# hello-robot/stretch_mujoco

Measured on AMD Instinct MI355X. Metric: env-steps/sec (whole node), 4096 parallel Stretch envs in total, higher is better.
Workload: dtype f32

## Files before the change

stretch_mujoco_amd/csrc/smj_builds.h:

```cpp
#pragma once
#define SMJ_BUILDS_INCLUDED 1

#define SMJ_BUILDS(X) \
  X(step) X(pgs) X(prof) X(tall) X(mid) X(midp) X(big38) X(big38p) X(big50) X(big50p) X(big) X(sat) X(sat1) X(sat2) X(satp) X(sat32) X(sat32n)
#define SMJ_CARRIES_NEWTON 1
#define SMJ_CARRIES_PGS 2
#define SMJ_CARRIES_BOTH 3
#define SMJ_FAM_STD 0
#define SMJ_FAM_TALL 1
#define SMJ_FAM_MID 2
#define SMJ_FAM_BIG38 3
#define SMJ_FAM_BIG50 4
#define SMJ_FAM_BIG 5
#define SMJ_FAM_SAT16 6
#define SMJ_FAM_SAT32 7
#define SMJ_ROW_step    SMJ_FAM_STD,   SMJ_CARRIES_NEWTON, SMJ_CARRIES_NEWTON, 1, 0, 0
#define SMJ_ROW_pgs     SMJ_FAM_STD,   SMJ_CARRIES_PGS,    SMJ_CARRIES_PGS,    1, 0, 0
#define SMJ_ROW_prof    SMJ_FAM_STD,   SMJ_CARRIES_BOTH,   SMJ_CARRIES_BOTH,   1, 0, 1
#define SMJ_ROW_tall    SMJ_FAM_TALL,  SMJ_CARRIES_BOTH,   SMJ_CARRIES_BOTH,   1, 1, 0
#define SMJ_ROW_mid     SMJ_FAM_MID,   SMJ_CARRIES_NEWTON, SMJ_CARRIES_BOTH,   1, 0, 0
#define SMJ_ROW_midp    SMJ_FAM_MID,   SMJ_CARRIES_PGS,    SMJ_CARRIES_PGS,    1, 0, 0
#define SMJ_ROW_big38   SMJ_FAM_BIG38, SMJ_CARRIES_NEWTON, SMJ_CARRIES_BOTH,   1, 0, 0
#define SMJ_ROW_big38p  SMJ_FAM_BIG38, SMJ_CARRIES_PGS,    SMJ_CARRIES_PGS,    1, 0, 0
#define SMJ_ROW_big50   SMJ_FAM_BIG50, SMJ_CARRIES_NEWTON, SMJ_CARRIES_BOTH,   1, 0, 0
#define SMJ_ROW_big50p  SMJ_FAM_BIG50, SMJ_CARRIES_PGS,    SMJ_CARRIES_PGS,    1, 0, 0
#define SMJ_ROW_big     SMJ_FAM_BIG,   SMJ_CARRIES_BOTH,   SMJ_CARRIES_BOTH,   1, 1, 0
#define SMJ_ROW_sat     SMJ_FAM_SAT16, SMJ_CARRIES_NEWTON, SMJ_CARRIES_NEWTON, 1, 0, 0
#define SMJ_ROW_sat1    SMJ_FAM_SAT16, SMJ_CARRIES_PGS,    SMJ_CARRIES_PGS,    1, 0, 0
#define SMJ_ROW_sat2    SMJ_FAM_SAT16, SMJ_CARRIES_NEWTON, SMJ_CARRIES_NEWTON, 2, 0, 0
#define SMJ_ROW_satp    SMJ_FAM_SAT16, SMJ_CARRIES_PGS,    SMJ_CARRIES_PGS,    2, 0, 0
#define SMJ_ROW_sat32   SMJ_FAM_SAT32, SMJ_CARRIES_BOTH,   SMJ_CARRIES_BOTH,   1, 1, 0
#define SMJ_ROW_sat32n  SMJ_FAM_SAT32, SMJ_CARRIES_NEWTON, SMJ_CARRIES_NEWTON, 2, 1, 0
#define smj_step_kernel_step smj_step_kernel
#define smj_launch_step_step smj_launch_step

#define SMJ_CAT2(a, b) a##b
#define SMJ_CAT(a, b) SMJ_CAT2(a, b)
#define SMJ_STR2(a) #a
#define SMJ_STR(a) SMJ_STR2(a)
#define SMJ_COLUMN(m, ...) m(__VA_ARGS__, ~)
#define SMJ_COL0(a, ...) a
#define SMJ_COL1(a, b, ...) b
#define SMJ_COL2(a, b, c, ...) c
#define SMJ_COL3(a, b, c, d, ...) d
#define SMJ_COL4(a, b, c, d, e, ...) e
#define SMJ_COL5(a, b, c, d, e, f, ...) f
#ifdef SMJ_BUILD_TAG
#define SMJ_BUILD_ROW SMJ_CAT(SMJ_ROW_, SMJ_BUILD_TAG)
#define SMJ_BUILD_FAM SMJ_COLUMN(SMJ_COL0, SMJ_BUILD_ROW)
#define SMJ_BUILD_WAVES SMJ_COLUMN(SMJ_COL3, SMJ_BUILD_ROW)
#define SMJ_STEP_KERNEL SMJ_CAT(smj_step_kernel_, SMJ_BUILD_TAG)
#define SMJ_LAUNCH_STEP SMJ_CAT(smj_launch_step_, SMJ_BUILD_TAG)
#if SMJ_COLUMN(SMJ_COL4, SMJ_BUILD_ROW)
#define SMJ_WORKER_KERNEL SMJ_CAT(SMJ_CAT(smj_step_kernel_, SMJ_BUILD_TAG), _worker)
#define SMJ_BUILD_WORKER_NAME SMJ_STR(SMJ_WORKER_KERNEL)
#else
#define SMJ_BUILD_WORKER_NAME nullptr
#endif
#else
#define SMJ_BUILD_FAM SMJ_FAM_STD
#endif

#if SMJ_BUILD_FAM == SMJ_FAM_STD
#define SMJ_BUILD_FAMILY "std"
#elif SMJ_BUILD_FAM == SMJ_FAM_TALL
#define SMJ_BUILD_FAMILY "tall"
#define SMJ_TALL 1
#elif SMJ_BUILD_FAM == SMJ_FAM_MID
#define SMJ_BUILD_FAMILY "mid"
#define SMJ_TALL 1
#define SMJ_TALL_ROWS 128
#define SMJ_TALL_CONTACTS 44
#elif SMJ_BUILD_FAM == SMJ_FAM_BIG38
// ... 84 lines not shown
```

stretch_mujoco_amd/csrc/smj_model.h:

```cpp
#pragma once
#include <stdint.h>

#include "smj_builds.h"
#if defined(SMJ_SAT)
#define NSAT SMJ_SAT
#define NVP 32
#ifndef SMJ_SAT_ROWS
#define SMJ_SAT_ROWS 320
#define SMJ_SAT_CONTACTS 64
#define SMJ_SAT_DENSE 256
#endif
#define NEFC SMJ_SAT_ROWS
#define NCON SMJ_SAT_CONTACTS
#define NDR SMJ_SAT_DENSE
#ifndef SMJ_SAT_EXT
#define SMJ_SAT_EXT 4
#endif
#ifndef SMJ_SAT_PGS
#define SMJ_SAT_PGS (SMJ_SAT_DENSE < 160 ? SMJ_SAT_DENSE : 160)
#endif
#define NXS SMJ_SAT_EXT
static_assert(NDR % 16 == 0 && NDR <= NEFC, "dense rows: whole 16-row blocks (matT_J, MFMA k-steps)");
#define NENT 5
#elif defined(SMJ_BIG)
// ... 87 lines not shown
  int nsat, nq_all, nv_all, nbody_all, nfric_main, nlimit_main;
  const int* k_satrec;
  int nsgeom, nstatpair, grid_dim[3];
  float grid_org[3], grid_h, grid_margin;
  const int* k_sgrec;
  const int* k_sprec;
  const int* k_spair;
  const int* k_grid_adr;
  const int* k_grid_list;
  const int* k_sg_cell;
  const float* k_sg_bound;
  const float* k_sgw;
#define X(n) const int* n;
  SMJ_MODEL_I32(X)
#undef X
#define X(n) const float* n;
  SMJ_MODEL_F32(X)
#undef X
  const int* k_lanerec;
  const int* k_pprec;
  const int* k_cgrec;
  const int* k_rowrec;
  const int* k_cprec;
};
enum { SMJ_CP_PAIR = 0, SMJ_CP_G1, SMJ_CP_G2, SMJ_CP_S1, SMJ_CP_S2, SMJ_CP_MARGIN, SMJ_CP_MG, SMJ_CP_CONDIM, SMJ_CP_FRIC = 8, SMJ_CP_SOLIMP = 13,
       SMJ_CP_SOLREF = 18, SMJ_CP_RBMIN = 20 ,
       SMJ_CP_B1 = 21, SMJ_CP_B2 = 22 , SMJ_CP_STRIDE = 24 };
enum { SMJ_RR_TYPE = 0, SMJ_RR_ID, SMJ_RR_D1, SMJ_RR_D2, SMJ_RR_Q1, SMJ_RR_Q2, SMJ_RR_V1, SMJ_RR_V2, SMJ_RR_DATA = 8, SMJ_RR_DIAG = 13,
       SMJ_RR_FLOSS = 14, SMJ_RR_SOLREF = 15, SMJ_RR_SOLIMP = 17, SMJ_RR_SAT = 22 , SMJ_RR_SDOF = 23 , SMJ_RR_STRIDE = 24 };
constexpr int smj_lr_act(int nent) { return 76 + ((7 * nent + 3) & ~3); }
constexpr int smj_lr_stride(int nent) { return smj_lr_act(nent) + 28; }
enum { SMJ_LR_KIN = 0, SMJ_LR_BODY = 36, SMJ_LR_DOF = 60, SMJ_LR_ENT = 76, SMJ_LR_ACT = smj_lr_act(NENT), SMJ_LR_STRIDE = smj_lr_stride(NENT) };
enum { SMJ_PP_PAIR = 0, SMJ_PP_G1, SMJ_PP_G2, SMJ_PP_B1, SMJ_PP_B2, SMJ_PP_T2, SMJ_PP_MARGIN, SMJ_PP_RBOUND2, SMJ_PP_BCEN2 = 8,
       SMJ_PP_POS1 = 11, SMJ_PP_MAT1 = 14, SMJ_PP_POS2 = 23, SMJ_PP_MAT2 = 26, SMJ_PP_SIZE2 = 35, SMJ_PP_CONDIM = 38, SMJ_PP_MG = 39,
       SMJ_PP_FRIC = 40, SMJ_PP_SOLIMP = 45, SMJ_PP_SOLREF = 50, SMJ_PP_BOX2 = 52 ,
       SMJ_PP_STRIDE = 60 };
enum { SMJ_CG_GEOM = 0, SMJ_CG_BODY, SMJ_CG_META, SMJ_CG_POS = 3, SMJ_CG_MAT = 6, SMJ_CG_LCEN = 15, SMJ_CG_HALF = 18, SMJ_CG_CCEN = 21,
       SMJ_CG_SIZE = 24, SMJ_CG_RBOUND = 27, SMJ_CG_STRIDE = 28 };

enum { SMJ_SR_BODY = 0, SMJ_SR_JTYPE, SMJ_SR_QADR, SMJ_SR_DADR, SMJ_SR_NDOF, SMJ_SR_JNT, SMJ_SR_F = 8,
       SMJ_SR_POS = SMJ_SR_F + 0, SMJ_SR_QUAT = SMJ_SR_F + 3, SMJ_SR_JPOS = SMJ_SR_F + 7, SMJ_SR_JAXIS = SMJ_SR_F + 10, SMJ_SR_Q0 = SMJ_SR_F + 13,
       SMJ_SR_INL = SMJ_SR_F + 14, SMJ_SR_ARM = SMJ_SR_F + 24, SMJ_SR_DAMP = SMJ_SR_F + 30, SMJ_SR_STIFF = SMJ_SR_F + 36, SMJ_SR_SPRING = SMJ_SR_F + 37,
       SMJ_SR_GCMASS = SMJ_SR_F + 38, SMJ_SR_GCIPOS = SMJ_SR_F + 39, SMJ_SR_STRIDE = 52 };
struct SmjStageLayout {
  int qpos, qvel, warm, ctrl, bctl, nstep, info, actlen, actvel, base, gyro, accel, xpose, stride;
};
constexpr SmjStageLayout smj_stage_layout(int nvp, int nbp, int nsat = 0) {
// ... 99 lines not shown
```

stretch_mujoco_amd/csrc/smj_model_load.h:

```cpp
#pragma once
#include <stdint.h>
#include <stdio.h>
#include <math.h>
#include <string.h>

#include <map>
#include <string>
#include <vector>

#include "../../include/smj.h"
#include "smj_model.h"

#define SMJ_SOLVER_OPTIONS(X)                                                                                                             \
  X("iterations", iterations, int) X("tolerance", tolerance, float) X("warmstart", warmstart, int) X("pgs_fixed_iter", pgs_fixed_iter, int) \
  X("qcqp_exact", qcqp_exact, int) X("grad_noise", grad_noise, float) X("pgs_island_stop", pgs_island_stop, int)                            \
  X("max_contacts_per_pair", max_con_pair, int) X("solver", solver, int) X("convex_pairs", convex_pairs, int) X("multiccd", multiccd, int)  \
  X("sep_cache", sep_cache, int) X("manifold_cache", manifold_cache, int) X("pgs_dual_warmstart", pgs_dual_ws, int)                         \
  X("", ls_iterations, int) X("", multi_serial, int) X("", ls_tolerance, float)
static inline bool smj_set_solver_option(DevModel& m, const char* name, double v) {
#define X(opt, field, type) if ((opt)[0] && !strcmp(name, opt)) { m.field = (type)v; return true; }
  SMJ_SOLVER_OPTIONS(X)
#undef X
  return false;
}
// ... 108 lines not shown
      for (int u = 0; u < nent; u++) {
        const int e = L + 64 * u, ok = e < m.nldl, ex = ok ? e : 0, i = gi("k_ldl_i", ex), j = gi("k_ldl_j", ex);
        k[u] = ok ? i : -1; k[nent + u] = ok ? j : 0; k[2 * nent + u] = fb((ok && i == j) ? gf("dof_armature", i) : 0.f);
        k[3 * nent + u] = ok ? gi("k_ldl_lact", ex) : -1;
        k[4 * nent + u] = fb(ok ? gf("k_ldl_damp", ex) : 0.f); k[5 * nent + u] = fb(ok ? gf("k_ldl_dcoef", ex) : 0.f); k[6 * nent + u] = fb(ok ? gf("k_ldl_lcoef", ex) : 0.f);
      }
    }
    {
      int* k = r + LR_ACT;
      const int a = L < nu ? L : 0;
      for (int u = 0; u < 4; u++) {
        const int dd = gi("k_act_dof", 4 * a + u);
        k[u] = L < nu ? dd : -1; k[4 + u] = dd >= 0 ? gi("k_dof_qposadr", dd) : 0; k[8 + u] = fb(gf("k_act_mom", 4 * a + u));
      }
      k[12] = fb(gf("actuator_gainprm", 3 * a));
      for (int q = 0; q < 3; q++) k[13 + q] = fb(gf("actuator_biasprm", 3 * a + q));
      k[16] = fb(gf("actuator_ctrlrange", 2 * a)); k[17] = fb(gf("actuator_ctrlrange", 2 * a + 1));
      k[18] = fb(gf("actuator_forcerange", 2 * a)); k[19] = fb(gf("actuator_forcerange", 2 * a + 1));
      k[20] = (gi("actuator_ctrllimited", a) ? 1 : 0) | (gi("actuator_forcelimited", a) ? 2 : 0) | (gi("actuator_biastype", a) == 1 ? 4 : 0);
      const int g = L < m.ngc ? gi("k_gc_body", L) : 0;
      k[21] = g; k[22] = gi("k_body_dofmask_lo", g); k[23] = gi("k_body_dofmask_hi", g);
      k[24] = fb(L < m.ngc ? gf("body_gcmass", g) : 0.f);
      for (int q = 0; q < 3; q++) k[25 + q] = fb(gf("body_gcipos", 3 * g + q));
    }
  }
  return rec;
}

static inline std::vector<int> smj_build_pprec(const DevModel& m, std::map<std::string, std::vector<int>>& I,
                                               std::map<std::string, std::vector<float>>& F) {
  std::vector<int> rec((size_t)(m.nplanepair > 0 ? m.nplanepair : 1) * SMJ_PP_STRIDE, 0);
  auto fb = [](float v) { int b; memcpy(&b, &v, 4); return b; };
  auto gi = [&](const char* n, size_t k) { const std::vector<int>& v = I[n]; return k < v.size() ? v[k] : 0; };
  auto gf = [&](const char* n, size_t k) { const std::vector<float>& v = F[n]; return k < v.size() ? v[k] : 0.f; };
  for (int t = 0; t < m.nplanepair; t++) {
    int* k = rec.data() + (size_t)t * SMJ_PP_STRIDE;
    const int p = gi("k_planepair", t), g1 = gi("pair_geom1", p), g2 = gi("pair_geom2", p);
    k[SMJ_PP_PAIR] = p; k[SMJ_PP_G1] = g1; k[SMJ_PP_G2] = g2; k[SMJ_PP_B1] = gi("geom_bodyid", g1); k[SMJ_PP_B2] = gi("geom_bodyid", g2);
    k[SMJ_PP_T2] = gi("geom_type", g2); k[SMJ_PP_MARGIN] = fb(gf("pair_margin", p)); k[SMJ_PP_RBOUND2] = fb(gf("geom_rbound", g2));
    for (int q = 0; q < 3; q++) {
      k[SMJ_PP_BCEN2 + q] = fb(gf("k_geom_bcenter", 3 * g2 + q));
      k[SMJ_PP_POS1 + q] = fb(gf("geom_pos", 3 * g1 + q)); k[SMJ_PP_POS2 + q] = fb(gf("geom_pos", 3 * g2 + q));
      k[SMJ_PP_SIZE2 + q] = fb(gf("geom_size", 3 * g2 + q));
    }
    for (int q = 0; q < 9; q++) { k[SMJ_PP_MAT1 + q] = fb(gf("k_geom_mat", 9 * g1 + q)); k[SMJ_PP_MAT2 + q] = fb(gf("k_geom_mat", 9 * g2 + q)); }
    k[SMJ_PP_CONDIM] = gi("pair_condim", p); k[SMJ_PP_MG] = fb(gf("pair_margin", p) - gf("pair_gap", p));
// ... 266 lines not shown
    const SmjBlobEntry* ei = b.find("k_sat_i");
    const SmjBlobEntry* ef = b.find("k_sat_f");
    if (!ei || !ef || ei->dtype != 1 || ef->dtype != 0 || ei->nbytes < 32u * m.nsat || ef->nbytes < 8u * 44u * m.nsat) { err = "model blob: satellite tables missing"; return -3; }
    std::vector<int> si(8 * (size_t)m.nsat), rec((size_t)m.nsat * SMJ_SR_STRIDE, 0);
    memcpy(si.data(), b.p + ei->offset, 32u * m.nsat);
    hosti["k_sat_i"] = si;
    const double* sf = reinterpret_cast<const double*>(b.p + ef->offset);
    for (int sidx = 0; sidx < m.nsat; sidx++) {
      int* k = rec.data() + (size_t)sidx * SMJ_SR_STRIDE;
      for (int q = 0; q < 8; q++) k[q] = si[8 * sidx + q];
      for (int q = 0; q < 44; q++) { const float v = (float)sf[44 * sidx + q]; memcpy(&k[SMJ_SR_F + q], &v, 4); }
    }
    m.k_satrec = up.i32(rec);
    if (!m.k_satrec) { err = "device allocation failed for k_satrec"; return -2; }
    m.nfric_main = 0;
    for (int f = 0; f < m.nfric; f++) m.nfric_main += hosti["k_fric_dof"][f] < m.nv;
    m.nlimit_main = 0;
    for (int L = 0; L < m.nlimit; L++) m.nlimit_main += hosti["jnt_dofadr"][hosti["k_limit_jnt"][L]] < m.nv;
  }
  {
    std::vector<int> rec = smj_build_lanerec(m, hosti, hostf, nent);
    m.k_lanerec = up.i32(rec);
    if (!m.k_lanerec) { err = "device allocation failed for k_lanerec"; return -2; }
    std::vector<int> pp = smj_build_pprec(m, hosti, hostf), cg = smj_build_cgrec(m, hosti, hostf);
    m.k_pprec = up.i32(pp);
    m.k_cgrec = up.i32(cg);
    if (!m.k_pprec || !m.k_cgrec) { err = "device allocation failed for the collision records"; return -2; }
    std::vector<int> rr = smj_build_rowrec(m, hosti, hostf);
    m.k_rowrec = up.i32(rr);
    if (!m.k_rowrec) { err = "device allocation failed for k_rowrec"; return -2; }
    std::vector<int> cp = smj_build_cprec(m, hosti, hostf);
    m.k_cprec = up.i32(cp);
    if (!m.k_cprec) { err = "device allocation failed for k_cprec"; return -2; }
  }
  return 0;
}
```

stretch_mujoco_amd/csrc/smj_step_impl.h:

```cpp
#pragma once
#ifndef SMJ_PROFILING
#define SMJ_PROFILING 1
#endif
#include <cstddef>
#include "smj_model.h"
#include "smj_wave.h"
#include "smj_sat_mem.h"

#define JS (NVS + 1)
#define MS (NVS + 1)
#define SMJ_MINVAL 1e-15f
#define SMJ_MINIMP 0.0001f
#define SMJ_MAXIMP 0.9999f

enum { JT_FREE = 0, JT_BALL = 1, JT_SLIDE = 2, JT_HINGE = 3 };
enum { GT_PLANE = 0, GT_SPHERE = 2, GT_CAPSULE = 3, GT_ELLIPSOID = 4, GT_CYLINDER = 5, GT_BOX = 6, GT_MESH = 7 };
enum { CT_EQUALITY = 0, CT_FRICTION = 1, CT_LIMIT = 3, CT_CONTACT_FRICTIONLESS = 5, CT_CONTACT_ELLIPTIC = 7, CT_NONE = -1 };

#if NSAT > 0
#define NCGS (NCG + 1)
#define NSURV 128
#else
#define NCGS NCG
#endif
// ... 239 lines not shown
    la = fmaxf(0.f, la + delta);
  }
#pragma unroll
  for (int i = 0; i < N; i++) res[i] *= dd[i];
  la_io = la;
  return la != 0;
}

SMJ_DEV float impedance(const float* solimp, float pos, float margin) {
  float dmin = fminf(SMJ_MAXIMP, fmaxf(SMJ_MINIMP, solimp[0])), dmax = fminf(SMJ_MAXIMP, fmaxf(SMJ_MINIMP, solimp[1]));
  float width = fmaxf(SMJ_MINVAL, solimp[2]), mid = fminf(SMJ_MAXIMP, fmaxf(SMJ_MINIMP, solimp[3])), power = fmaxf(1.0f, solimp[4]);
  if (dmin == dmax) return 0.5f * (dmin + dmax);
  float x = fabsf(pos - margin) / width, y;
  if (x >= 1) return dmax;
  if (x <= 0) return dmin;
  if (power == 1.0f) y = x;
  else if (power == 2.0f) y = (x <= mid) ? x * x / mid : 1 - (1 - x) * (1 - x) / (1 - mid);
  else if (x <= mid) y = powf(x, power) / powf(mid, power - 1);
  else y = 1 - powf(1 - x, power) / powf(1 - mid, power - 1);
  return dmin + y * (dmax - dmin);
}

#ifdef SMJ_EMUL
static long smj_emul_sep_skips = 0;
static long smj_emul_ext_steps = 0;
static long smj_emul_mc_hits = 0;
static long smj_emul_isl_total = 0, smj_emul_isl_swept = 0;
#endif
struct StepKernel {
  const DevModel& M;
  const DevState& S;
  Smem& s;
  int env;

  PL<float[6]> cdof, cdof_dot;
  PL<float> qvel_r, g_r, qacc_r;
  PL<float> f_r[NPS], r_r[NPS], ARinv_r[NPS];
  PL<float> qla_r;
  int nefc, ncon, niter, flags;
  float* ppc = nullptr;
  int step_base = 0;
  int pipe_chunk = 0;
  bool parked = false;
  bool split_on = false, rev = false;
  bool serial_redo = false;

// ... 3121 lines not shown
    LANES { if (lane == 0) s.sat.nch = 0; }
#endif
    SYNC();
    ROWS_BEGIN(rb, ne) LANES {
      float c = 0, f = 0;
      int st = 0;
      const int i = lane + rb, t = nr.type[lane];
      const float jar = nr.jar[lane], D = nr.D[lane], R = nr.R[lane];
      if (i < ne) {
        if (t == CT_EQUALITY) { f = -D * jar; st = 1; c = 0.5f * D * jar * jar; }
        else if (t == CT_FRICTION) {
          const float fl = nr.fl[lane];
          if (jar <= -R * fl) { f = fl; st = 2; c = -fl * (0.5f * R * fl + jar); }
          else if (jar >= R * fl) { f = -fl; st = 3; c = -fl * (0.5f * R * fl - jar); }
          else { f = -D * jar; st = 1; c = 0.5f * D * jar * jar; }
        } else if (t == CT_LIMIT || t == CT_CONTACT_FRICTIONLESS) {
          if (jar < 0) { f = -D * jar; st = 1; c = 0.5f * D * jar * jar; }
        }
      }
      nr.force[lane] = f; nr.state[lane] = st; cost[lane] += c;
      if (i < NEFC) s.ef[i] = f;
    } ROWS_END_RW(rb)
    SYNC();
    ROWS_BEGIN(rb, ne) LANES {
      const int c = nr.c0[lane];
      if (c >= 0) {
        const int i = lane + rb, dim = s.cdim[c];
        const float mu = nr.cq[lane][6];
        float U[6], jr[6], S[6], Rj[6], T = 0;
#pragma unroll
        for (int j = 0; j < 6; j++) {
          const int jj = j < dim ? j : 0;
          jr[j] = s.eb[i + jj];
          Rj[j] = s.eR[i + jj];
          S[j] = j == 0 ? mu : (j < dim ? s.cfric[c][j - 1] : 0.f);
          U[j] = jr[j] * S[j];
          if (j > 0) T += U[j] * U[j];
        }
        const float N = U[0];
        const float Tinv = T > 0 ? fast_rsqrt(T) : 0.f;
        T = T * Tinv;
        int st;
        float cc = 0, ef[6] = {0, 0, 0, 0, 0, 0};
        if (N >= mu * T || (T <= 0 && N >= 0)) { st = 0; }
        else if (mu * N + T <= 0 || (T <= 0 && N < 0)) {
          st = 1;
#pragma unroll
          for (int j = 0; j < 6; j++)
            if (j < dim) { const float Dj = fast_rcp(Rj[j]); ef[j] = -Dj * jr[j]; cc += 0.5f * Dj * jr[j] * jr[j]; }
        } else {
          st = 4;
          const float Dm = nr.cq[lane][5], NT = N - mu * T, Ti = Tinv;
          cc = 0.5f * Dm * NT * NT;
          const float fn = -Dm * NT * mu;
          ef[0] = fn;
#pragma unroll
          for (int j = 1; j < 6; j++) ef[j] = -fn * Ti * U[j] * S[j];
#if NSAT > 0
          const int hslot = want_hess ? lds_atomic_inc(&s.sat.nch) : NCH;
          s.sat.chs[c] = hslot < NCH ? (signed char)hslot : (signed char)-1;
          if (want_hess && hslot < NCH) {
            float* H = s.u.n.cH[hslot];
#else
          if (want_hess) {
            float* H = s.u.n.cH[c];
#endif
            const float a = mu * N * Ti * Ti * Ti, b = mu * NT * Ti;
            H[0] = Dm * S[0] * S[0];
#pragma unroll
            for (int j = 1; j < 6; j++) H[j] = H[6 * j] = -mu * U[j] * Ti * Dm * S[0] * S[j];
#pragma unroll
            for (int j = 1; j < 6; j++)
#pragma unroll
              for (int k = 1; k < 6; k++) H[6 * j + k] = (a * U[j] * U[k] - (j == k ? b : 0.f)) * Dm * S[j] * S[k];
          }
        }
        cost[lane] += cc;
#pragma unroll
        for (int j = 0; j < 6; j++)
          if (j < dim) { s.ef[i + j] = ef[j]; s.estate[i + j] = st; }
      }
    } ROWS_END_RO()
    SYNC();
    ROWS_BEGIN(rb, ne) LANES {
      const int i = lane + rb;
      if (i < NEFC) {
        if (nr.type[lane] == CT_CONTACT_ELLIPTIC && i < ne) { nr.force[lane] = s.ef[i]; nr.state[lane] = s.estate[i]; }
        s.estate[i] = (i < ne) ? nr.state[lane] : 0;
      }
    } ROWS_END_RW(rb)
    return wave_sum(cost);
  }

#ifdef SMJ_EMUL
  struct F2 { float x, y; };
  static inline void pk_fma(F2& acc, float a0, float a1, float b0, float b1) { acc.x += a0 * b0; acc.y += a1 * b1; }
#else
  typedef float F2 __attribute__((ext_vector_type(2)));
  SMJ_DEV static void pk_fma(F2& acc, float a0, float a1, float b0, float b1) {
    const F2 a = {a0, a1}, b = {b0, b1};
    acc = acc + a * b;
  }
#endif
// ... 147 lines not shown
    } else if constexpr (J < N) {
      PL<float> cj;
      LANES { cj[lane] = hrow[lane][J]; }
      const float hkj = wave_read(cj, K);
      LANES { hrow[lane][J] -= mult[lane] * hkj; }
    }
  }
  template <int K, int N>
  SMJ_DEV void gj_cols(PL<float[NVS]>& hrow, PL<float>& x, PL<float>& pinv, const PL<int>& ol) {
    if constexpr (K < N) {
      PL<float> col, mult;
      LANES { col[lane] = hrow[lane][K]; }
      const float rp = fast_rcp(fmaxf(wave_read(col, K), 1e-30f));
      LANES {
        mult[lane] = ol[lane] == K ? 0.f : col[lane] * rp;
        if (ol[lane] == K) pinv[lane] = rp;
      }
      gj_pair<K, K + 1, N>(hrow, mult);
      const float xk = wave_read(x, K);
      LANES { x[lane] -= mult[lane] * xk; }
      gj_cols<K + 1, N>(hrow, x, pinv, ol);
    }
  }
  template <int N>
  SMJ_DEV void gj_solve(PL<float>& x) {
    PL<float[NVS]> hrow;
    PL<float> pinv;
    PL<int> ol;
    LANES { ol[lane] = opaque(lane); }
    LANES {
      const int i = NVS == 32 ? (lane & 31) : (lane < NVS ? lane : NVS - 1);
#pragma unroll
      for (int k = 0; k < N; k++) hrow[lane][k] = s.u.n.H[i][k];
      pinv[lane] = 0.f;
      if (lane >= N) x[lane] = 0.f;
    }
    gj_cols<0, N>(hrow, x, pinv, ol);
    LANES { x[lane] *= pinv[lane]; }
  }
  SMJ_DEV void gj_solve_lds(PL<float>& x) {
    const int n = M.nv;
    LANES { if (lane < NVS) s.u.n.H[lane][NVS] = lane < n ? x[lane] : 0.f; }
    SYNC();
    for (int k = 0; k < n; k++) {
      const float rp = fast_rcp(fmaxf(uni(s.u.n.H[k][k]), 1e-30f));
      LANES {
        if (lane < n && lane != k) {
          float* row = s.u.n.H[lane];
          const float* piv = s.u.n.H[k];
          const float mult = row[k] * rp;
          int j = k + 1;
          for (; j + 8 <= n; j += 8) {
            float a[8], b[8];
#pragma unroll
            for (int u = 0; u < 8; u++) { a[u] = row[j + u]; b[u] = piv[j + u]; }
#pragma unroll
            for (int u = 0; u < 8; u++) row[j + u] = a[u] - mult * b[u];
          }
          for (; j < n; j++) row[j] -= mult * piv[j];
          row[NVS] -= mult * piv[NVS];
        }
      }
      SYNC();
    }
    LANES { x[lane] = lane < n ? s.u.n.H[lane][NVS] * fast_rcp(fmaxf(s.u.n.H[lane][lane], 1e-30f)) : 0.f; }
    SYNC();
  }
  SMJ_DEV void solve_H(PL<float>& x, bool rare = false) {
#if NVP == 32
    if (M.nv <= 26) gj_solve<26>(x);
    else gj_solve<NVP>(x);
#else
    if (rare || M.nv > 50) gj_solve_lds(x);
#if NVS >= 50
    else if (M.nv > 38) gj_solve<50>(x);
#endif
    else gj_solve<38>(x);
#endif
  }

  SMJ_DEV float ls_eval(NRow& nr0, const float* qg, float a, float& d1, float& d2) {
    const int ne = nefc;
    PL<float> p0, p1, p2;
    LANES { p0[lane] = 0.f; p1[lane] = 0.f; p2[lane] = 0.f; }
    ROWS_BEGIN(rb, ne) LANES {
      float c0 = 0, c1 = 0, c2 = 0;
      if (lane + rb < ne) {
        const int t = nr.type[lane];
        const float x = nr.jar[lane] + a * nr.jv[lane];
        if (t == CT_EQUALITY) { c0 = nr.q0[lane]; c1 = nr.q1[lane]; c2 = nr.q2[lane]; }
        else if (t == CT_FRICTION) {
          const float fl = nr.fl[lane], rf = nr.R[lane] * fl;
          if (x <= -rf) { c0 = fl * (-0.5f * rf - nr.jar[lane]); c1 = -fl * nr.jv[lane]; }
          else if (x >= rf) { c0 = fl * (-0.5f * rf + nr.jar[lane]); c1 = fl * nr.jv[lane]; }
          else { c0 = nr.q0[lane]; c1 = nr.q1[lane]; c2 = nr.q2[lane]; }
        } else if (t == CT_LIMIT || t == CT_CONTACT_FRICTIONLESS) {
          if (x < 0) { c0 = nr.q0[lane]; c1 = nr.q1[lane]; c2 = nr.q2[lane]; }
        } else if (nr.c0[lane] >= 0) {
          const float* k = nr.cq[lane];
          const float mu = k[6], Dm = k[5], N = k[0] + a * k[1], Tsq = k[2] + a * (2 * k[3] + a * k[4]);
          if (Tsq <= 0) { if (N < 0) { c0 = nr.q0[lane]; c1 = nr.q1[lane]; c2 = nr.q2[lane]; } }
          else {
            const float Ti = fast_rsqrt(Tsq), T = Tsq * Ti;
            if (N >= mu * T) {}
            else if (mu * N + T <= 0) { c0 = nr.q0[lane]; c1 = nr.q1[lane]; c2 = nr.q2[lane]; }
            else {
              const float w = k[3] + a * k[4], N1 = k[1], T1 = w * Ti, T2 = k[4] * Ti - w * w * Ti * Ti * Ti;
              const float NT = N - mu * T, NT1 = N1 - mu * T1;
              const float v = 0.5f * Dm * NT * NT, g = Dm * NT * NT1, h = Dm * (NT1 * NT1 - NT * mu * T2);
              c2 = 0.5f * h; c1 = g - h * a; c0 = v - a * g + 0.5f * h * a * a;
            }
          }
        }
      }
      p0[lane] += c0; p1[lane] += c1; p2[lane] += c2;
    } ROWS_END_RO()
    const float q0 = qg[0] + wave_sum(p0), q1 = qg[1] + wave_sum(p1), q2 = qg[2] + wave_sum(p2);
    d1 = 2 * a * q2 + q1;
    d2 = 2 * q2;
    return a * a * q2 + a * q1 + q0;
  }
// ... 22 lines not shown
#endif
      }
      niter = 0;
      SYNC();
      return;
    }
    ROWS_BEGIN_(rb, ne, false) LANES {
      const int row = lane + rb;
      float vel = 0;
      const bool on = row < ne;
      if (on) {
        const float* jr = jrow(row);
        for (int k = 0; k < nv; k++) vel += jr[k] * s.qvel[k];
#if NSAT > 0
        vel += sat_jdot(row, SX_V);
#endif
      }
      nr.type[lane] = on ? s.etype[row] : CT_NONE;
      nr.R[lane] = on ? s.eR[row] : 1.f;
      nr.D[lane] = on ? 1.0f / s.eR[row] : 0.f;
      nr.fl[lane] = on ? s.efloss[row] : 0.f;
      nr.aref[lane] = on ? -s.eBv[row] * vel - s.eK[row] * s.eimp[row] * (s.epos[row] - s.emargin[row]) : 0.f;
      int c0 = -1;
      if (on && s.etype[row] == CT_CONTACT_ELLIPTIC && s.cefc[s.eid[row]] == row) c0 = s.eid[row];
      nr.c0[lane] = c0;
      nr.state[lane] = 0; nr.jar[lane] = 0.f; nr.jv[lane] = 0.f; nr.force[lane] = 0.f; nr.q0[lane] = 0.f; nr.q1[lane] = 0.f; nr.q2[lane] = 0.f;
      for (int k = 0; k < 7; k++) nr.cq[lane][k] = 0.f;
      if (c0 >= 0) {
        const float mu = contact_mu(c0);
        nr.cq[lane][6] = mu;
        nr.cq[lane][5] = (1.0f / s.eR[row]) / fmaxf(mu * mu * (1 + mu * mu), SMJ_MINVAL);
      }
      if (dbg && row < NEFC) s.earef[row] = nr.aref[lane];
    } ROWS_END_RW(rb)
#if NSAT > 0
    const int nvt = M.nv_all;
#else
    const int nvt = nv;
#endif
    const float scale = 1.0f / (M.meaninertia * (float)(nvt > 1 ? nvt : 1));
    LANES { qacc[lane] = (lane < nv && M.warmstart) ? s.warm[lane] : 0.f; }
    mat_M(Ma, qacc);
#if NSAT > 0
    if (!M.warmstart) { LANES { if (lane >= 32 && lane - 32 < M.nsat) for (int k = 0; k < 6; k++) s.sat.x[SX_QA][lane - 32][k] = 0.f; } }
    sat_matM(SX_MA, SX_QA);
    SYNC();
#endif
    ROWS_BEGIN(rb, ne) mat_J_exact(nr.jar, qacc, nr.aref, rb); ROWS_END_RW(rb)
    float cost = 0;
    TICK(SMJ_PROF_WARM)
    int iter = 0;
    bool at_update = false;
    for (; iter < M.iterations;) {
      TICK(SMJ_PROF_PGS)
// ... 91 lines not shown
                  for (int t = 0; t < NT; t++) b[t][lane][ks] = s.J[k][16 * t + c];
                }
              }
            }
#pragma unroll
            for (int ks = 0; ks < KB; ks++) {
              if (kb + ks < ksteps && kb + ks < NDR / 4) {
                PL<float> pa[NT], pb[NT];
                LANES {
#pragma unroll
                  for (int t = 0; t < NT; t++) { pb[t][lane] = b[t][lane][ks]; pa[t][lane] = wk[lane][ks] * pb[t][lane]; }
                }
#pragma unroll
                for (int ta = 0; ta < NT; ta++)
#pragma unroll
                  for (int tb = 0; tb <= ta; tb++) mfma16x16x4(acc[ta * (ta + 1) / 2 + tb], pa[ta], pb[tb]);
              }
            }
          }
        }
        long long th = 0;
        if (prof) { th = smj_clock(); pc[SMJ_PROF_H_K] += (float)(th - t0); }
        int nks = 0;
        for (uint64_t cm = conemask; cm;) {
          const int c = ffs64(cm);
          cm &= cm - 1;
          const int r0 = uni(s.cefc[c]), dim = uni(s.cdim[c]);
          if (r0 >= ndense()) continue;
          for (int q0 = 0; q0 < dim; q0 += 4) {
            nks++;
            PL<float> pa[NT], pb[NT];
            LANES {
              const int q = q0 + (lane >> 4), col = lane & 15, qc = q < 6 ? q : 5;
              const float on = q < dim ? 1.f : 0.f;
              float hq[6];
#if NSAT > 0
              const int hc = s.sat.chs[c];
#else
              const int hc = c;
#endif
#pragma unroll
              for (int p = 0; p < 6; p++) hq[p] = on * s.u.n.cH[hc][6 * qc + p];
#pragma unroll
              for (int t = 0; t < NT; t++) {
                float jv[6], av = 0.f;
#pragma unroll
// ... 88 lines not shown
          a1[lane] = lane < nv ? search[lane] * (Ma[lane] - g_r[lane]) : 0.f;
          a2[lane] = lane < nv ? 0.5f * search[lane] * Mv[lane] : 0.f;
#if NSAT > 0
          if (lane >= 32 && lane - 32 < M.nsat) {
            const int si = lane - 32;
            for (int k = 0; k < 6; k++) {
              a1[lane] += s.sat.x[SX_SRCH][si][k] * (s.sat.x[SX_MA][si][k] - s.sat.x[SX_G][si][k]);
              a2[lane] += 0.5f * s.sat.x[SX_SRCH][si][k] * s.sat.x[SX_MV][si][k];
            }
          }
#endif
        }
        qg[0] = gauss; qg[1] = wave_sum(a1); qg[2] = wave_sum(a2);
      }
      ROWS_BEGIN(rb, ne) LANES {
        const int row = lane + rb;
        const float D = nr.D[lane], ja = nr.jar[lane], jv = nr.jv[lane];
        nr.q0[lane] = 0.5f * D * ja * ja; nr.q1[lane] = D * ja * jv; nr.q2[lane] = 0.5f * D * jv * jv;
        if (row < NEFC) { s.eb[row] = ja; s.ef[row] = jv; s.earef[row] = nr.q0[lane]; s.eK[row] = nr.q1[lane]; s.eBv[row] = nr.q2[lane]; }
      } ROWS_END_RW(rb)
      SYNC();
      ROWS_BEGIN(rb, ne) LANES {
        const int c = nr.c0[lane];
        if (c >= 0) {
          const int i = lane + rb, dim = s.cdim[c];
          float a0 = 0, a1 = 0, a2 = 0, uu = 0, uv = 0, vv = 0;
#pragma unroll
          for (int j = 1; j < 6; j++) {
            const int jj = j < dim ? j : 1;
            const float on = j < dim ? 1.f : 0.f;
            a0 += on * s.earef[i + jj]; a1 += on * s.eK[i + jj]; a2 += on * s.eBv[i + jj];
            const float fr = on * s.cfric[c][jj - 1], u = s.eb[i + jj] * fr, v = s.ef[i + jj] * fr;
            uu += u * u; uv += u * v; vv += v * v;
          }
          nr.q0[lane] += a0; nr.q1[lane] += a1; nr.q2[lane] += a2;
          const float mu = nr.cq[lane][6];
          nr.cq[lane][0] = nr.jar[lane] * mu; nr.cq[lane][1] = nr.jv[lane] * mu;
          nr.cq[lane][2] = uu; nr.cq[lane][3] = uv; nr.cq[lane][4] = vv;
        }
      } ROWS_END_RW(rb)
      TICK(SMJ_PROF_N_PREP)
      float alpha = 0, d10 = 0;
      {
        const float gtol = M.tolerance * M.ls_tolerance * snorm * M.meaninertia * (float)(nvt > 1 ? nvt : 1);
        float d1, d2, lo = 0, hi = -1;
        {
          PL<float> gs;
// ... 97 lines not shown
      for (int t = 0; t < NENT; t++) {
        const int i = et.i[lane][t], j = et.j[lane][t];
        if (i < 0) continue;
        float v = (i == j) ? s.Mdiag[i] : s.MM[j][i];
        if (implicit) {
          float d = et.damp[lane][t] - et.dcoef[lane][t];
          const int la = et.lact[lane][t];
          if (la >= 0) d -= et.lcoef[lane][t] * s.act_free[la];
          v += h * d;
        }
        s.u.n.H[i][j] = v;
        s.u.n.H[j][i] = v;
      }
    }
    SYNC();
  }

  SMJ_DEV void integrate() {
    const int nv = M.nv;
    const float h = M.timestep;
#if SMJ_W2_INTEGRATE
    fork2(W2_SAT_INTEGRATE);
#endif
    build_dense(true);
    PL<float> x;
    LANES { x[lane] = lane < nv ? s.tmp[lane] : 0.f; }
    solve_H(x);
    LANES {
      if (lane < nv) s.qvel[lane] += h * x[lane];
    }
    SYNC();
    LANES {
      if (lane < M.njnt) {
        const int j = lane, qa = M.jnt_qposadr[j], da = M.jnt_dofadr[j];
        if (M.jnt_type[j] == JT_FREE) {
          for (int k = 0; k < 3; k++) s.qpos[qa + k] += h * s.qvel[da + k];
          float wv[3] = {s.qvel[da + 3], s.qvel[da + 4], s.qvel[da + 5]};
          const float nrm = sqrtf(dot3(wv, wv)), ang = nrm * h;
          float q[4] = {s.qpos[qa + 3], s.qpos[qa + 4], s.qpos[qa + 5], s.qpos[qa + 6]};
          if (ang > 0) {
            const float sn = sinf(0.5f * ang) / nrm, dq[4] = {cosf(0.5f * ang), wv[0] * sn, wv[1] * sn, wv[2] * sn};
            quat_mul(q, q, dq);
          }
          quat_normalize(q);
          for (int k = 0; k < 4; k++) s.qpos[qa + 3 + k] = q[k];
        } else s.qpos[qa] += h * s.qvel[da];
      }
    }
    SYNC();
    PL<int> bad;
// ... 248 lines not shown
```

Measured before the change: 12.97 million.

## Batch cone Hessian MFMA k-steps across contacts, fill cone Hessian by rows, direct-integrate from MM

Adds a per-build cone-batch column (set to 4 for step, prof and mid). When it is above one, the Newton cone-Hessian accumulation gathers several contacts per group and issues their MFMA k-steps together, instead of looping one contact at a time. The cone Hessian blocks are filled in parallel by friction rows (encoding row index in c0), rather than one lane writing all 36 entries. Integration can skip build_dense by patching only the implicit damping entries of the mass matrix in place, solving from it, and restoring them, driven by a new host-built per-row sparse record. This adds register pressure, more complex encoding, and a new device table.

```diff
diff --git a/stretch_mujoco_amd/csrc/smj_builds.h b/stretch_mujoco_amd/csrc/smj_builds.h
--- a/stretch_mujoco_amd/csrc/smj_builds.h
+++ b/stretch_mujoco_amd/csrc/smj_builds.h
@@ -14,23 +14,23 @@
 #define SMJ_FAM_BIG 5
 #define SMJ_FAM_SAT16 6
 #define SMJ_FAM_SAT32 7
-#define SMJ_ROW_step    SMJ_FAM_STD,   SMJ_CARRIES_NEWTON, SMJ_CARRIES_NEWTON, 1, 0, 0
-#define SMJ_ROW_pgs     SMJ_FAM_STD,   SMJ_CARRIES_PGS,    SMJ_CARRIES_PGS,    1, 0, 0
-#define SMJ_ROW_prof    SMJ_FAM_STD,   SMJ_CARRIES_BOTH,   SMJ_CARRIES_BOTH,   1, 0, 1
-#define SMJ_ROW_tall    SMJ_FAM_TALL,  SMJ_CARRIES_BOTH,   SMJ_CARRIES_BOTH,   1, 1, 0
-#define SMJ_ROW_mid     SMJ_FAM_MID,   SMJ_CARRIES_NEWTON, SMJ_CARRIES_BOTH,   1, 0, 0
-#define SMJ_ROW_midp    SMJ_FAM_MID,   SMJ_CARRIES_PGS,    SMJ_CARRIES_PGS,    1, 0, 0
-#define SMJ_ROW_big38   SMJ_FAM_BIG38, SMJ_CARRIES_NEWTON, SMJ_CARRIES_BOTH,   1, 0, 0
-#define SMJ_ROW_big38p  SMJ_FAM_BIG38, SMJ_CARRIES_PGS,    SMJ_CARRIES_PGS,    1, 0, 0
-#define SMJ_ROW_big50   SMJ_FAM_BIG50, SMJ_CARRIES_NEWTON, SMJ_CARRIES_BOTH,   1, 0, 0
-#define SMJ_ROW_big50p  SMJ_FAM_BIG50, SMJ_CARRIES_PGS,    SMJ_CARRIES_PGS,    1, 0, 0
-#define SMJ_ROW_big     SMJ_FAM_BIG,   SMJ_CARRIES_BOTH,   SMJ_CARRIES_BOTH,   1, 1, 0
-#define SMJ_ROW_sat     SMJ_FAM_SAT16, SMJ_CARRIES_NEWTON, SMJ_CARRIES_NEWTON, 1, 0, 0
-#define SMJ_ROW_sat1    SMJ_FAM_SAT16, SMJ_CARRIES_PGS,    SMJ_CARRIES_PGS,    1, 0, 0
-#define SMJ_ROW_sat2    SMJ_FAM_SAT16, SMJ_CARRIES_NEWTON, SMJ_CARRIES_NEWTON, 2, 0, 0
-#define SMJ_ROW_satp    SMJ_FAM_SAT16, SMJ_CARRIES_PGS,    SMJ_CARRIES_PGS,    2, 0, 0
-#define SMJ_ROW_sat32   SMJ_FAM_SAT32, SMJ_CARRIES_BOTH,   SMJ_CARRIES_BOTH,   1, 1, 0
-#define SMJ_ROW_sat32n  SMJ_FAM_SAT32, SMJ_CARRIES_NEWTON, SMJ_CARRIES_NEWTON, 2, 1, 0
+#define SMJ_ROW_step    SMJ_FAM_STD,   SMJ_CARRIES_NEWTON, SMJ_CARRIES_NEWTON, 1, 0, 0, 4
+#define SMJ_ROW_pgs     SMJ_FAM_STD,   SMJ_CARRIES_PGS,    SMJ_CARRIES_PGS,    1, 0, 0, 1
+#define SMJ_ROW_prof    SMJ_FAM_STD,   SMJ_CARRIES_BOTH,   SMJ_CARRIES_BOTH,   1, 0, 1, 4
+#define SMJ_ROW_tall    SMJ_FAM_TALL,  SMJ_CARRIES_BOTH,   SMJ_CARRIES_BOTH,   1, 1, 0, 1
+#define SMJ_ROW_mid     SMJ_FAM_MID,   SMJ_CARRIES_NEWTON, SMJ_CARRIES_BOTH,   1, 0, 0, 4
+#define SMJ_ROW_midp    SMJ_FAM_MID,   SMJ_CARRIES_PGS,    SMJ_CARRIES_PGS,    1, 0, 0, 1
+#define SMJ_ROW_big38   SMJ_FAM_BIG38, SMJ_CARRIES_NEWTON, SMJ_CARRIES_BOTH,   1, 0, 0, 1
+#define SMJ_ROW_big38p  SMJ_FAM_BIG38, SMJ_CARRIES_PGS,    SMJ_CARRIES_PGS,    1, 0, 0, 1
+#define SMJ_ROW_big50   SMJ_FAM_BIG50, SMJ_CARRIES_NEWTON, SMJ_CARRIES_BOTH,   1, 0, 0, 1
+#define SMJ_ROW_big50p  SMJ_FAM_BIG50, SMJ_CARRIES_PGS,    SMJ_CARRIES_PGS,    1, 0, 0, 1
+#define SMJ_ROW_big     SMJ_FAM_BIG,   SMJ_CARRIES_BOTH,   SMJ_CARRIES_BOTH,   1, 1, 0, 1
+#define SMJ_ROW_sat     SMJ_FAM_SAT16, SMJ_CARRIES_NEWTON, SMJ_CARRIES_NEWTON, 1, 0, 0, 1
+#define SMJ_ROW_sat1    SMJ_FAM_SAT16, SMJ_CARRIES_PGS,    SMJ_CARRIES_PGS,    1, 0, 0, 1
+#define SMJ_ROW_sat2    SMJ_FAM_SAT16, SMJ_CARRIES_NEWTON, SMJ_CARRIES_NEWTON, 2, 0, 0, 1
+#define SMJ_ROW_satp    SMJ_FAM_SAT16, SMJ_CARRIES_PGS,    SMJ_CARRIES_PGS,    2, 0, 0, 1
+#define SMJ_ROW_sat32   SMJ_FAM_SAT32, SMJ_CARRIES_BOTH,   SMJ_CARRIES_BOTH,   1, 1, 0, 1
+#define SMJ_ROW_sat32n  SMJ_FAM_SAT32, SMJ_CARRIES_NEWTON, SMJ_CARRIES_NEWTON, 2, 1, 0, 1
 #define smj_step_kernel_step smj_step_kernel
 #define smj_launch_step_step smj_launch_step
 
@@ -45,10 +45,14 @@
 #define SMJ_COL3(a, b, c, d, ...) d
 #define SMJ_COL4(a, b, c, d, e, ...) e
 #define SMJ_COL5(a, b, c, d, e, f, ...) f
+#define SMJ_COL6(a, b, c, d, e, f, g, ...) g
 #ifdef SMJ_BUILD_TAG
 #define SMJ_BUILD_ROW SMJ_CAT(SMJ_ROW_, SMJ_BUILD_TAG)
 #define SMJ_BUILD_FAM SMJ_COLUMN(SMJ_COL0, SMJ_BUILD_ROW)
 #define SMJ_BUILD_WAVES SMJ_COLUMN(SMJ_COL3, SMJ_BUILD_ROW)
+#ifndef SMJ_CONE_CB
+#define SMJ_CONE_CB SMJ_COLUMN(SMJ_COL6, SMJ_BUILD_ROW)
+#endif
 #define SMJ_STEP_KERNEL SMJ_CAT(smj_step_kernel_, SMJ_BUILD_TAG)
 #define SMJ_LAUNCH_STEP SMJ_CAT(smj_launch_step_, SMJ_BUILD_TAG)
 #if SMJ_COLUMN(SMJ_COL4, SMJ_BUILD_ROW)
diff --git a/stretch_mujoco_amd/csrc/smj_model.h b/stretch_mujoco_amd/csrc/smj_model.h
--- a/stretch_mujoco_amd/csrc/smj_model.h
+++ b/stretch_mujoco_amd/csrc/smj_model.h
@@ -133,7 +133,10 @@
   const int* k_cgrec;
   const int* k_rowrec;
   const int* k_cprec;
-};
+  const int* k_imprec;
+  int imp_nslot;
+};
+enum { SMJ_IR_N = 8, SMJ_IR_STRIDE = 5 * SMJ_IR_N };
 enum { SMJ_CP_PAIR = 0, SMJ_CP_G1, SMJ_CP_G2, SMJ_CP_S1, SMJ_CP_S2, SMJ_CP_MARGIN, SMJ_CP_MG, SMJ_CP_CONDIM, SMJ_CP_FRIC = 8, SMJ_CP_SOLIMP = 13,
        SMJ_CP_SOLREF = 18, SMJ_CP_RBMIN = 20 ,
        SMJ_CP_B1 = 21, SMJ_CP_B2 = 22 , SMJ_CP_STRIDE = 24 };
diff --git a/stretch_mujoco_amd/csrc/smj_model_load.h b/stretch_mujoco_amd/csrc/smj_model_load.h
--- a/stretch_mujoco_amd/csrc/smj_model_load.h
+++ b/stretch_mujoco_amd/csrc/smj_model_load.h
@@ -154,6 +154,31 @@
       k[21] = g; k[22] = gi("k_body_dofmask_lo", g); k[23] = gi("k_body_dofmask_hi", g);
       k[24] = fb(L < m.ngc ? gf("body_gcmass", g) : 0.f);
       for (int q = 0; q < 3; q++) k[25 + q] = fb(gf("body_gcipos", 3 * g + q));
+    }
+  }
+  return rec;
+}
+
+static inline std::vector<int> smj_build_imprec(const DevModel& m, std::map<std::string, std::vector<int>>& I,
+                                                std::map<std::string, std::vector<float>>& F, int& nslot) {
+  std::vector<int> rec(64 * SMJ_IR_STRIDE, 0);
+  auto fb = [](float v) { int b; memcpy(&b, &v, 4); return b; };
+  auto gi = [&](const char* n, size_t k) { const std::vector<int>& v = I[n]; return k < v.size() ? v[k] : 0; };
+  auto gf = [&](const char* n, size_t k) { const std::vector<float>& v = F[n]; return k < v.size() ? v[k] : 0.f; };
+  for (int L = 0; L < 64; L++)
+    for (int u = 0; u < SMJ_IR_N; u++) { rec[L * SMJ_IR_STRIDE + u] = -1; rec[L * SMJ_IR_STRIDE + SMJ_IR_N + u] = -1; }
+  int used[64] = {0};
+  nslot = 0;
+  for (int e = 0; e < m.nldl; e++) {
+    const int i = gi("k_ldl_i", e), j = gi("k_ldl_j", e), la = gi("k_ldl_lact", e);
+    const float damp = gf("k_ldl_damp", e), dcoef = gf("k_ldl_dcoef", e), lcoef = gf("k_ldl_lcoef", e);
+    if (damp == 0.f && dcoef == 0.f && la < 0) continue;
+    for (int side = 0; side < (i == j ? 1 : 2); side++) {
+      const int row = side ? j : i, col = side ? i : j;
+      if (row < 0 || row >= m.nv || row >= 64 || used[row] >= SMJ_IR_N) { nslot = -1; return rec; }
+      int* k = rec.data() + row * SMJ_IR_STRIDE + used[row]++;
+      k[0] = col; k[SMJ_IR_N] = la; k[2 * SMJ_IR_N] = fb(damp); k[3 * SMJ_IR_N] = fb(dcoef); k[4 * SMJ_IR_N] = fb(lcoef);
+      if (used[row] > nslot) nslot = used[row];
     }
   }
   return rec;
@@ -466,6 +491,9 @@
     std::vector<int> rec = smj_build_lanerec(m, hosti, hostf, nent);
     m.k_lanerec = up.i32(rec);
     if (!m.k_lanerec) { err = "device allocation failed for k_lanerec"; return -2; }
+    std::vector<int> ir = smj_build_imprec(m, hosti, hostf, m.imp_nslot);
+    m.k_imprec = up.i32(ir);
+    if (!m.k_imprec) { err = "device allocation failed for k_imprec"; return -2; }
     std::vector<int> pp = smj_build_pprec(m, hosti, hostf), cg = smj_build_cgrec(m, hosti, hostf);
     m.k_pprec = up.i32(pp);
     m.k_cgrec = up.i32(cg);
diff --git a/stretch_mujoco_amd/csrc/smj_step_impl.h b/stretch_mujoco_amd/csrc/smj_step_impl.h
--- a/stretch_mujoco_amd/csrc/smj_step_impl.h
+++ b/stretch_mujoco_amd/csrc/smj_step_impl.h
@@ -285,6 +285,21 @@
 }
 
 #ifdef SMJ_EMUL
+#undef SMJ_CONE_CB
+#define SMJ_CONE_CB (NVP == 32 ? 4 : 2)
+#elif !defined(SMJ_CONE_CB)
+#define SMJ_CONE_CB 1
+#endif
+static_assert(SMJ_CONE_CB == 1 || SMJ_CONE_CB % 2 == 0, "a group is whole contacts: two k-steps each");
+#define SMJ_NEWTON_BATCHED (SMJ_CONE_CB > 1)
+#define SMJ_CH_ROWS (SMJ_NEWTON_BATCHED && NSAT == 0)
+#ifdef SMJ_EMUL
+extern "C" {
+int smj_emul_serial_newton = 0;
+long smj_emul_cone_group_ksteps = 0;
+long smj_emul_ch_row_fills = 0;
+long smj_emul_direct_integrations = 0;
+}
 static long smj_emul_sep_skips = 0;
 static long smj_emul_ext_steps = 0;
 static long smj_emul_mc_hits = 0;
@@ -3452,11 +3467,17 @@
       if (i < NEFC) s.ef[i] = f;
     } ROWS_END_RW(rb)
     SYNC();
+#if SMJ_CH_ROWS && defined(SMJ_EMUL)
+    const bool by_rows = want_hess && !smj_emul_serial_newton;
+#else
+    const bool by_rows = SMJ_CH_ROWS && want_hess;
+#endif
     ROWS_BEGIN(rb, ne) LANES {
-      const int c = nr.c0[lane];
-      if (c >= 0) {
-        const int i = lane + rb, dim = s.cdim[c];
+      const int cj = nr.c0[lane];
+      if (cj >= 0 && (cj < 256 || by_rows)) {
+        const int c = cj & 255, j = cj >> 8, i = lane + rb - j, dim = s.cdim[c];
         const float mu = nr.cq[lane][6];
+        const float So = j == 0 ? mu : s.cfric[c][j > 0 ? j - 1 : 0], Uo = s.eb[lane + rb < NEFC ? lane + rb : 0] * So;
         float U[6], jr[6], S[6], Rj[6], T = 0;
 #pragma unroll
         for (int j = 0; j < 6; j++) {
@@ -3496,6 +3517,21 @@
             float* H = s.u.n.cH[c];
 #endif
             const float a = mu * N * Ti * Ti * Ti, b = mu * NT * Ti;
+#if SMJ_CH_ROWS
+            if (by_rows) {
+#ifdef SMJ_EMUL
+              smj_emul_ch_row_fills++;
+#endif
+              H[6 * j] = j == 0 ? Dm * S[0] * S[0] : -mu * Uo * Ti * Dm * S[0] * So;
+#pragma unroll
+              for (int k = 1; k < 6; k++)
+                H[6 * j + k] = j == 0 ? -mu * U[k] * Ti * Dm * S[0] * S[k] : (a * Uo * U[k] - (j == k ? b : 0.f)) * Dm * So * S[k];
+              if (j + dim < 6)
+#pragma unroll
+                for (int k = 0; k < 6; k++) H[6 * (j + dim) + k] = 0.f;
+            } else
+#endif
+            {
             H[0] = Dm * S[0] * S[0];
 #pragma unroll
             for (int j = 1; j < 6; j++) H[j] = H[6 * j] = -mu * U[j] * Ti * Dm * S[0] * S[j];
@@ -3503,12 +3539,15 @@
             for (int j = 1; j < 6; j++)
 #pragma unroll
               for (int k = 1; k < 6; k++) H[6 * j + k] = (a * U[j] * U[k] - (j == k ? b : 0.f)) * Dm * S[j] * S[k];
+            }
           }
         }
-        cost[lane] += cc;
-#pragma unroll
-        for (int j = 0; j < 6; j++)
-          if (j < dim) { s.ef[i + j] = ef[j]; s.estate[i + j] = st; }
+        if (j == 0) {
+          cost[lane] += cc;
+#pragma unroll
+          for (int r = 0; r < 6; r++)
+            if (r < dim) { s.ef[i + r] = ef[r]; s.estate[i + r] = st; }
+        }
       }
     } ROWS_END_RO()
     SYNC();
@@ -3702,7 +3741,7 @@
       gj_cols<K + 1, N>(hrow, x, pinv, ol);
     }
   }
-  template <int N>
+  template <int N, bool FROM_M = false>
   SMJ_DEV void gj_solve(PL<float>& x) {
     PL<float[NVS]> hrow;
     PL<float> pinv;
@@ -3711,7 +3750,7 @@
     LANES {
       const int i = NVS == 32 ? (lane & 31) : (lane < NVS ? lane : NVS - 1);
 #pragma unroll
-      for (int k = 0; k < N; k++) hrow[lane][k] = s.u.n.H[i][k];
+      for (int k = 0; k < N; k++) hrow[lane][k] = FROM_M ? s.MM[i][k] : s.u.n.H[i][k];
       pinv[lane] = 0.f;
       if (lane >= N) x[lane] = 0.f;
     }
@@ -3746,16 +3785,18 @@
     LANES { x[lane] = lane < n ? s.u.n.H[lane][NVS] * fast_rcp(fmaxf(s.u.n.H[lane][lane], 1e-30f)) : 0.f; }
     SYNC();
   }
+  SMJ_DEV bool in_registers() const { return NVP == 32 || M.nv <= 50; }
+  template <bool FROM_M = false>
   SMJ_DEV void solve_H(PL<float>& x, bool rare = false) {
 #if NVP == 32
-    if (M.nv <= 26) gj_solve<26>(x);
-    else gj_solve<NVP>(x);
+    if (M.nv <= 26) gj_solve<26, FROM_M>(x);
+    else gj_solve<NVP, FROM_M>(x);
 #else
     if (rare || M.nv > 50) gj_solve_lds(x);
 #if NVS >= 50
-    else if (M.nv > 38) gj_solve<50>(x);
-#endif
-    else gj_solve<38>(x);
+    else if (M.nv > 38) gj_solve<50, FROM_M>(x);
+#endif
+    else gj_solve<38, FROM_M>(x);
 #endif
   }
 
@@ -3776,7 +3817,7 @@
           else { c0 = nr.q0[lane]; c1 = nr.q1[lane]; c2 = nr.q2[lane]; }
         } else if (t == CT_LIMIT || t == CT_CONTACT_FRICTIONLESS) {
           if (x < 0) { c0 = nr.q0[lane]; c1 = nr.q1[lane]; c2 = nr.q2[lane]; }
-        } else if (nr.c0[lane] >= 0) {
+        } else if ((unsigned)nr.c0[lane] < 256u) {
           const float* k = nr.cq[lane];
           const float mu = k[6], Dm = k[5], N = k[0] + a * k[1], Tsq = k[2] + a * (2 * k[3] + a * k[4]);
           if (Tsq <= 0) { if (N < 0) { c0 = nr.q0[lane]; c1 = nr.q1[lane]; c2 = nr.q2[lane]; } }
@@ -3845,14 +3886,18 @@
       nr.fl[lane] = on ? s.efloss[row] : 0.f;
       nr.aref[lane] = on ? -s.eBv[row] * vel - s.eK[row] * s.eimp[row] * (s.epos[row] - s.emargin[row]) : 0.f;
       int c0 = -1;
-      if (on && s.etype[row] == CT_CONTACT_ELLIPTIC && s.cefc[s.eid[row]] == row) c0 = s.eid[row];
+      if (on && s.etype[row] == CT_CONTACT_ELLIPTIC) {
+        const int c = s.eid[row], j = row - s.cefc[c];
+        if (j == 0) c0 = c;
+        else if (SMJ_CH_ROWS) c0 = c | (j << 8);
+      }
       nr.c0[lane] = c0;
       nr.state[lane] = 0; nr.jar[lane] = 0.f; nr.jv[lane] = 0.f; nr.force[lane] = 0.f; nr.q0[lane] = 0.f; nr.q1[lane] = 0.f; nr.q2[lane] = 0.f;
       for (int k = 0; k < 7; k++) nr.cq[lane][k] = 0.f;
       if (c0 >= 0) {
-        const float mu = contact_mu(c0);
+        const float mu = contact_mu(c0 & 255);
         nr.cq[lane][6] = mu;
-        nr.cq[lane][5] = (1.0f / s.eR[row]) / fmaxf(mu * mu * (1 + mu * mu), SMJ_MINVAL);
+        nr.cq[lane][5] = (1.0f / s.eR[row - (c0 >> 8)]) / fmaxf(mu * mu * (1 + mu * mu), SMJ_MINVAL);
       }
       if (dbg && row < NEFC) s.earef[row] = nr.aref[lane];
     } ROWS_END_RW(rb)
@@ -3990,6 +4035,91 @@
         long long th = 0;
         if (prof) { th = smj_clock(); pc[SMJ_PROF_H_K] += (float)(th - t0); }
         int nks = 0;
+#ifdef SMJ_EMUL
+        const bool grouped = SMJ_CONE_CB > 1 && !smj_emul_serial_newton;
+#else
+        constexpr bool grouped = SMJ_CONE_CB > 1;
+#endif
+        if (grouped) {
+          constexpr int CG = SMJ_CONE_CB > 1 ? SMJ_CONE_CB / 2 : 1;
+          PL<int> ent, cin;
+          LANES {
+            int e = 0, in = 0;
+            if (lane < NCON && ((conemask >> lane) & 1)) {
+              const int r0 = s.cefc[lane];
+#if NSAT > 0
+              const int hc = s.sat.chs[lane];
+#else
+              const int hc = lane;
+#endif
+              in = r0 < ndense();
+              e = r0 | (s.cdim[lane] << 12) | (hc << 16);
+            }
+            ent[lane] = e; cin[lane] = in;
+          }
+          for (uint64_t cm = wave_ballot(cin); cm;) {
+            int r0[CG], dim[CG], hc[CG];
+#pragma unroll
+            for (int g = 0; g < CG; g++) {
+              const int e = wave_read(ent, cm ? ffs64(cm) : 0);
+              r0[g] = e & 0xfff; dim[g] = cm ? (e >> 12) & 15 : 0; hc[g] = e >> 16;
+              cm &= cm - 1;
+            }
+            PL<float[6]> hq[CG][2], jv[CG][NT];
+            PL<float> jq[CG][2][NT], pa[CG][2][NT], pb[CG][2][NT];
+            LANES {
+              const int col = lane & 15;
+#pragma unroll
+              for (int g = 0; g < CG; g++) {
+#pragma unroll
+                for (int h = 0; h < 2; h++) {
+                  const int q = 4 * h + (lane >> 4), qc = q < 6 ? q : 5;
+#pragma unroll
+                  for (int p = 0; p < 6; p++) hq[g][h][lane][p] = s.u.n.cH[hc[g]][6 * qc + p];
+#pragma unroll
+                  for (int t = 0; t < NT; t++) jq[g][h][t][lane] = s.J[r0[g] + qc < NDR ? r0[g] + qc : NDR - 1][16 * t + col];
+                }
+#pragma unroll
+                for (int t = 0; t < NT; t++)
+#pragma unroll
+                  for (int p = 0; p < 6; p++) jv[g][t][lane][p] = s.J[r0[g] + p < NDR ? r0[g] + p : NDR - 1][16 * t + col];
+              }
+            }
+            LANES {
+#pragma unroll
+              for (int g = 0; g < CG; g++)
+#pragma unroll
+                for (int h = 0; h < 2; h++) {
+                  const float on = 4 * h + (lane >> 4) < dim[g] ? 1.f : 0.f;
+                  float hv[6];
+#pragma unroll
+                  for (int p = 0; p < 6; p++) hv[p] = on * hq[g][h][lane][p];
+#pragma unroll
+                  for (int t = 0; t < NT; t++) {
+                    float av = 0.f;
+#pragma unroll
+                    for (int p = 0; p < 6; p++) av += hv[p] * jv[g][t][lane][p];
+                    pa[g][h][t][lane] = av;
+                    pb[g][h][t][lane] = on * jq[g][h][t][lane];
+                  }
+                }
+            }
+#pragma unroll
+            for (int g = 0; g < CG; g++)
+#pragma unroll
+              for (int h = 0; h < 2; h++)
+                if (4 * h < dim[g]) {
+                  nks++;
+#pragma unroll
+                  for (int ta = 0; ta < NT; ta++)
+#pragma unroll
+                    for (int tb = 0; tb <= ta; tb++) mfma16x16x4(acc[ta * (ta + 1) / 2 + tb], pa[g][h][ta], pb[g][h][tb]);
+                }
+          }
+#ifdef SMJ_EMUL
+          smj_emul_cone_group_ksteps += nks;
+#endif
+        } else
         for (uint64_t cm = conemask; cm;) {
           const int c = ffs64(cm);
           cm &= cm - 1;
@@ -4124,7 +4254,7 @@
       SYNC();
       ROWS_BEGIN(rb, ne) LANES {
         const int c = nr.c0[lane];
-        if (c >= 0) {
+        if ((unsigned)c < 256u) {
           const int i = lane + rb, dim = s.cdim[c];
           float a0 = 0, a1 = 0, a2 = 0, uu = 0, uv = 0, vv = 0;
 #pragma unroll
@@ -4268,10 +4398,50 @@
 #if SMJ_W2_INTEGRATE
     fork2(W2_SAT_INTEGRATE);
 #endif
-    build_dense(true);
     PL<float> x;
     LANES { x[lane] = lane < nv ? s.tmp[lane] : 0.f; }
-    solve_H(x);
+    bool direct = SMJ_NEWTON_BATCHED && newton() && in_registers() && M.imp_nslot >= 0;
+#ifdef SMJ_EMUL
+    direct = direct && !smj_emul_serial_newton;
+#endif
+    if (direct) {
+#ifdef SMJ_EMUL
+      smj_emul_direct_integrations++;
+#endif
+      const int nslot = M.imp_nslot;
+      PL<int[SMJ_IR_N]> col;
+      PL<float[SMJ_IR_N]> old;
+      LANES {
+        const int* r = static_cast<const int*>(__builtin_assume_aligned(M.k_imprec + opaque(lane) * SMJ_IR_STRIDE, 16));
+#pragma unroll
+        for (int t = 0; t < SMJ_IR_N; t++) {
+          col[lane][t] = -1; old[lane][t] = 0.f;
+          if (t < nslot) {
+            const int c = r[t], la = r[SMJ_IR_N + t];
+            const float damp = asf(r[2 * SMJ_IR_N + t]), dcoef = asf(r[3 * SMJ_IR_N + t]), lcoef = asf(r[4 * SMJ_IR_N + t]);
+            col[lane][t] = c;
+            if (c >= 0) {
+              float v = s.MM[lane][c];
+              old[lane][t] = v;
+              float d = damp - dcoef;
+              if (la >= 0) d -= lcoef * s.act_free[la];
+              v += h * d;
+              s.MM[lane][c] = v;
+            }
+          }
+        }
+      }
+      SYNC();
+      solve_H<true>(x);
+      LANES {
+#pragma unroll
+        for (int t = 0; t < SMJ_IR_N; t++)
+          if (t < nslot && col[lane][t] >= 0) s.MM[lane][col[lane][t]] = old[lane][t];
+      }
+    } else {
+      build_dense(true);
+      solve_H(x);
+    }
     LANES {
       if (lane < nv) s.qvel[lane] += h * x[lane];
     }
```

New measurement: 12.99 million (median of 2 runs). No clear change (+0.2%).
